# tatsuki1107/Relevance-FactorizationMachine

Hardware: AMD Instinct MI355X
Metric: training examples/sec (FM, k=32) (higher is better)
Workload: dtype f64; 1 GPU; kuairec_big: synthetic KuaiRec-big-shaped log 7176x10728 + 110 side-feature columns, n_features=18014, 15 nnz/row, N_train=1000000, FM k=32, IPS, lr=9e-06, batch_size=65536 rows per GPU (global 65536), step = gather+forward+residual+gradients+SGD update; row-id lists precomputed; batch_size_per_gpu=65536, global_batch=65536, parallelism=single

## Files before the change

relevance_factorizationmachine_amd/csrc/rfm_fm_kernels.hpp:

```cpp
#pragma once

#include <hip/amd_detail/amd_hip_unsafe_atomics.h>
#include <hip/hip_runtime.h>

#include <cstdint>
#include <type_traits>

#include "rfm_device_utils.hpp"
#include "rfm_fm_records.h"

namespace rfm {

template <int BLOCK>
__device__ inline double block_sum(double v, double* lds) {
  const int tid = threadIdx.x;
  __syncthreads();
  lds[tid] = v;
  __syncthreads();
#pragma unroll
  for (int s = BLOCK / 2; s > 0; s >>= 1) {
    if (tid < s) lds[tid] += lds[tid + s];
    __syncthreads();
  }
  return lds[0];
}

__device__ inline double logloss_term(double y, double p, double pred, double eps) {
  const double r = y / p;
  return r * log(pred + eps) + (1.0 - r) * log(1.0 - pred + eps);
}

constexpr int kBigBlock = 1024;
constexpr int kBigWaves = 4;
constexpr int kFwdRows = 2;

constexpr int kBigUnroll = 3;
constexpr int kSmallUnroll = 8;
constexpr int kSmallWideUnroll = 2;

constexpr int rows_in_flight(int nc) { return nc == 1 ? kFwdRows : 1; }
constexpr int kFwdRowsPlain = kFwdRows;
constexpr int kPlainUnroll = kBigUnroll;
constexpr int rows_in_flight_plain(int nc) { return nc == 1 ? kFwdRowsPlain : 1; }

constexpr bool hot_fixed_order(int lpr, int nc, int block, int rows) {
  return nc == 1 && (block / lpr) * rows <= 128;
}
constexpr int kHotUnroll = 2;
constexpr int kHotPosPad = 4;
inline size_t forward_lds_bytes(int block, int lpr, int vec, int nc, int rows, int n_hot, int k,
                                bool fixed_order) {
  size_t bytes = size_t(block) * 8 + (size_t(block) * rows + size_t(block / lpr)) * sizeof(Entry) +
                 size_t(n_hot) * size_t(k + 2) * 8;
  if (block == kBigBlock && n_hot == 0) bytes += 2 * size_t(block / lpr) * rows * 24;
  if (fixed_order && n_hot > 0 && hot_fixed_order(lpr, nc, block, rows)) {
    const size_t rt = size_t(block / lpr) * rows;
    bytes += rt * size_t(lpr * vec) * 8;
    if (rt / 32 > 1) bytes += size_t(block / lpr) * size_t(k + 2) * 8;
    bytes += ((size_t(n_hot) * ((rt + 31) / 32) + 1) & ~size_t(1)) * 4;
    bytes += (size_t(n_hot) * (rt + kHotPosPad) + 7) / 8 * 8;
  }
  return bytes;
}

struct FwdArgs {
  const Entry* ent;
  const RowRec* rows;
  const char* ell;
  int64_t ell_stride;
  const double2* ell_yp;
  const int64_t* indptr;
  const int32_t* indices;
  const double* values;
  const double* y;
  const double* pscore;
  const int32_t* row_ids;
  int64_t n_rows;
  int64_t n_rows_a;
  const int64_t* indptr2;
  const int32_t* indices2;
  const double* values2;
  const double* y2;
  const double* pscore2;
  double* loss_partial2;
  const double* w0;
  const double* w;
  const double* V;
  int32_t k;
  double* out_pred;
  double* out_err;
  double* out_Q;
  SlotMark* slot_mark;
  unsigned long long* slot_bits;
  int32_t n_hot;
  int32_t hot_rounds;
  int32_t hot_fixed;
  double* hot_slab;
  double* err_partial;
  double* loss_partial;
  double eps;
  int32_t grid_main;
  const int32_t* row_ids_x;
  int64_t n_rows_x;
  double* out_pred_x;
  int32_t grid_x;
  const RowRec* rows_y;
  const Entry* ent_y;
  int64_t n_rows_y;
  double* out_pred_y;
};

struct HotEnt {
  int32_t off;
  int32_t pad;
  double coef;
};
static_assert(sizeof(HotEnt) == sizeof(Entry), "HotEnt replaces an Entry in place");

template <int LPR, int VEC, int NC, int BLOCK, int R, bool REC, bool ELL = false, bool DET = false,
          bool SEG = false, bool XTRA = false>
__global__ __launch_bounds__(BLOCK, (BLOCK == kBigBlock ? kBigWaves : 1)) void fm_forward_kernel(
    FwdArgs a) {
  constexpr int GPB = BLOCK / LPR;
  unsigned bx = blockIdx.x, gx = gridDim.x;
  if constexpr (XTRA && REC) {
    if (int(blockIdx.x) >= a.grid_main) {
      const bool second = int(blockIdx.x) >= a.grid_main + a.grid_x;
      bx = blockIdx.x - a.grid_main - (second ? a.grid_x : 0);
      gx = second ? gridDim.x - a.grid_main - a.grid_x : a.grid_x;
      a.row_ids = second ? nullptr : a.row_ids_x;
      a.n_rows = second ? a.n_rows_y : a.n_rows_x;
      if (second) {
        a.rows = a.rows_y;
        a.ent = a.ent_y;
      }
      a.n_hot = 0;
      a.slot_mark = nullptr;
      a.slot_bits = nullptr;
      a.out_Q = nullptr;
      a.out_err = nullptr;
      a.err_partial = nullptr;
      a.loss_partial = nullptr;
      a.out_pred = second ? a.out_pred_y : a.out_pred_x;
    } else {
      gx = a.grid_main;
    }
  }
  constexpr bool seg = SEG && !REC;
  extern __shared__ double dyn_lds[];
  const int tid = threadIdx.x;
  const int l = tid % LPR;
  const int g = tid / LPR;
  const int k = a.k;
  const int hot_w = k + 2;
  const int H = a.n_hot;
  double* red = dyn_lds;
  Entry* ebuf = reinterpret_cast<Entry*>(dyn_lds + BLOCK) + g * (R * LPR + 1);
  double* hot = dyn_lds + BLOCK + 2 * (BLOCK * R + GPB);
  constexpr bool FIX = DET && REC && hot_fixed_order(LPR, NC, BLOCK, R);
  constexpr int RT = GPB * R;
  constexpr int KS = LPR * VEC;
  constexpr int NW = (RT + 31) / 32;
  constexpr int NCELL = RT / 32 > 1 ? RT / 32 : 1;
  constexpr int NHV = NCELL > 1 ? GPB / NCELL : 0;
  constexpr int PS = RT + kHotPosPad;
  double* Qs = hot + H * hot_w;
  double* part = Qs + RT * KS;
  unsigned int* hbits = reinterpret_cast<unsigned int*>(part + (NCELL > 1 ? GPB * hot_w : 0));
  uint8_t* hpos = reinterpret_cast<uint8_t*>(hbits + ((H * NW + 1) & ~1));
  const double w0 = a.w0[0];
  const int64_t last_row = a.n_rows - 1;
  double loss_acc = 0.0, loss_acc2 = 0.0, err_acc = 0.0;
  const bool stage_loss = BLOCK == kBigBlock && a.loss_partial != nullptr && H == 0;
  double* lstage = hot;
  int trip = 0;
  int fo[NC];
  bool fok[NC];
#pragma unroll
  for (int c = 0; c < NC; ++c) {
    const int f = (c * LPR + l) * VEC;
    fok[c] = f < k;
    fo[c] = fok[c] ? f : 0;
  }

  if (H > 0) {
    for (int i = tid; i < H * hot_w; i += BLOCK) hot[i] = 0.0;
    if (FIX)
      for (int i = tid; i < H * NW; i += BLOCK) hbits[i] = 0u;
    __syncthreads();
  }
  for (int64_t base = int64_t(bx) * (GPB * R); base < a.n_rows;
       base += int64_t(gx) * (GPB * R)) {
    int64_t t[R];
    int32_t r[R];
    using EntryOff = typename std::conditional<REC, int32_t, int64_t>::type;
    EntryOff p0[R];
    int len[R];
    double yy[R], pp[R];
    bool valid[R];
#pragma unroll
    for (int i = 0; i < R; ++i) {
      t[i] = base + i * GPB + g;
      valid[i] = t[i] <= last_row;
      r[i] = int32_t(valid[i] ? t[i] : last_row);
    }
    bool sb[R];
#pragma unroll
    for (int i = 0; i < R; ++i) sb[i] = seg && (valid[i] ? t[i] : last_row) >= a.n_rows_a;
    if (a.row_ids) {
#pragma unroll
      for (int i = 0; i < R; ++i) r[i] = a.row_ids[sb[i] ? 0 : r[i]];
    }
    if constexpr (seg) {
#pragma unroll
      for (int i = 0; i < R; ++i)
        if (sb[i]) r[i] = int32_t((valid[i] ? t[i] : last_row) - a.n_rows_a);
    }
    int32_t nxt[R];
    const int64_t nbase = base + int64_t(gx) * (GPB * R);
    constexpr bool ell = REC && ELL;
    const bool warm = ell && BLOCK == kBigBlock && a.row_ids && nbase < a.n_rows;
    int32_t* parked = reinterpret_cast<int32_t*>(red);
    if (warm) {
#pragma unroll
      for (int i = 0; i < R; ++i) {
        const int64_t nt = nbase + i * GPB + g;
        nxt[i] = a.row_ids[nt <= last_row ? nt : last_row];
      }
    }
    Entry e0[R];
    if (ell) {
#pragma unroll
      for (int i = 0; i < R; ++i) {
        e0[i] = reinterpret_cast<const Entry*>(a.ell + int64_t(r[i]) * a.ell_stride)[l];
        const double2 yp = a.ell_yp[r[i]];
        yy[i] = yp.x;
        pp[i] = yp.y;
        p0[i] = 0;
      }
      constexpr int GPW = kWave / LPR;
#pragma unroll
      for (int i = 0; i < R; ++i) {
        unsigned long long live = __ballot(e0[i].slot != kNilSlot);
        if (GPW > 1) live = (live >> ((g % GPW) * LPR)) & ((1ull << (LPR % 64)) - 1ull);
        len[i] = valid[i] ? __popcll(live) : 0;
      }
    }
#pragma unroll
    for (int i = 0; i < R; ++i) {
      if (ell) {
      } else if (REC) {
        const RowRec rec = a.rows[r[i]];
        p0[i] = EntryOff(rec.begin);
        len[i] = valid[i] ? int(rec.len) : 0;
        yy[i] = rec.y;
        pp[i] = rec.p;
      } else {
        const int64_t* ip = sb[i] ? a.indptr2 : a.indptr;
        const int64_t b0 = ip[r[i]], b1 = ip[r[i] + 1];
        p0[i] = EntryOff(b0);
        len[i] = valid[i] ? int(b1 - b0) : 0;
        yy[i] = 0.0;
        pp[i] = 1.0;
      }
    }
    if (!REC && a.y) {
#pragma unroll
      for (int i = 0; i < R; ++i) {
        yy[i] = (sb[i] ? a.y2 : a.y)[r[i]];
        pp[i] = (sb[i] ? a.pscore2 : a.pscore)[r[i]];
      }
    }
    int maxlen = len[0];
#pragma unroll
    for (int i = 1; i < R; ++i) maxlen = max(maxlen, len[i]);
    if (warm) {
#pragma unroll
      for (int i = 0; i < R; ++i)
        if (l == 0) parked[i * GPB + g] = nxt[i];
    }

    double q[R][NC][VEC];
    double s2[R], lin[R], err[R];
#pragma unroll
    for (int i = 0; i < R; ++i) {
      s2[i] = 0.0;
      lin[i] = 0.0;
      err[i] = 0.0;
#pragma unroll
      for (int c = 0; c < NC; ++c)
#pragma unroll
        for (int v = 0; v < VEC; ++v) q[i][c][v] = 0.0;
    }

    for (int pb = 0; pb < maxlen; pb += LPR) {
      Entry e[R];
#pragma unroll
      for (int i = 0; i < R; ++i) {
        const int my = pb + l;
        const EntryOff at = len[i] > 0 ? p0[i] + min(my, len[i] - 1) : 0;
        if (ell) {
          e[i] = e0[i];
        } else if (REC) {
          e[i] = a.ent[at];
        } else {
          e[i].col = (sb[i] ? a.indices2 : a.indices)[at];
          e[i].slot = 0;
          e[i].x = (sb[i] ? a.values2 : a.values)[at];
        }
        if (my >= len[i]) {
          e[i].slot = 0;
          e[i].x = 0.0;
        }
      }
#pragma unroll
      for (int i = 0; i < R; ++i) {
        lin[i] += a.w[e[i].col] * e[i].x;
        ebuf[i * LPR + l] = e[i];
      }
      const int cnt = (maxlen - pb) < LPR ? (maxlen - pb) : LPR;
#pragma unroll(BLOCK == kBigBlock || NC > 1 ? (NC == 1 && !DET && (ELL || !REC) ? (REC ? kBigUnroll : kPlainUnroll) : (BLOCK == kBigBlock || NC > 4 ? 2 : kSmallWideUnroll)) : kSmallUnroll)
      for (int j = 0; j < cnt; ++j) {
        Entry ej[R];
        Pack<VEC> pv[R][NC];
#pragma unroll
        for (int i = 0; i < R; ++i) {
          ej[i] = ebuf[i * LPR + j];
          const double* vrow = a.V + int64_t(ej[i].col) * k;
#pragma unroll
          for (int c = 0; c < NC; ++c) pv[i][c].load(vrow + fo[c]);
        }
#pragma unroll
        for (int i = 0; i < R; ++i) {
#pragma unroll
          for (int c = 0; c < NC; ++c) {
            const double xm = fok[c] ? ej[i].x : 0.0;
#pragma unroll
            for (int v = 0; v < VEC; ++v) {
              const double vx = pv[i][c].v[v] * xm;
              q[i][c][v] += vx;
              s2[i] += vx * vx;
            }
          }
        }
      }
    }

    if (warm) {
#pragma unroll
      for (int i = 0; i < R; ++i) nxt[i] = parked[i * GPB + g];
    }
#pragma unroll
    for (int i = 0; i < R; ++i) asm volatile("" ::"v"(yy[i]), "v"(pp[i]));
#pragma unroll
    for (int i = 0; i < R; ++i) {
      if (len[i] == 0) {
        s2[i] = 0.0;
        lin[i] = 0.0;
#pragma unroll
        for (int c = 0; c < NC; ++c)
#pragma unroll
          for (int v = 0; v < VEC; ++v) q[i][c][v] = 0.0;
      }
      double pair = -s2[i];
#pragma unroll
      for (int c = 0; c < NC; ++c)
#pragma unroll
        for (int v = 0; v < VEC; ++v) pair += q[i][c][v] * q[i][c][v];
      pair = group_sum<LPR>(pair);
      const double linsum = group_sum<LPR>(lin[i]);
      const double pred = sigmoid_clipped(w0 + linsum + 0.5 * pair);
      err[i] = valid[i] ? yy[i] / pp[i] - pred : 0.0;
      if (valid[i]) {
        if (a.out_Q) {
          const uint32_t qoff = uint32_t(t[i]) * uint32_t(k);
#pragma unroll
          for (int c = 0; c < NC; ++c) {
            if (fok[c]) {
              Pack<VEC> pq;
#pragma unroll
              for (int v = 0; v < VEC; ++v) pq.v[v] = q[i][c][v];
              if (REC)
                pq.store_through(a.out_Q + (qoff + uint32_t(fo[c])));
              else
                pq.store(a.out_Q + (qoff + uint32_t(fo[c])));
            }
          }
        }
        if (l == 0) {
          if (a.out_pred) a.out_pred[t[i]] = pred;
          if (a.out_err) a.out_err[t[i]] = err[i];
          if (a.loss_partial) {
            if (stage_loss) {
              double* st = lstage + ((trip & 1) * RT + i * GPB + g) * 3;
              st[0] = pred;
              st[1] = yy[i];
              st[2] = pp[i];
            } else if (sb[i]) {
              loss_acc2 += logloss_term(yy[i], pp[i], pred, a.eps);
            } else {
              loss_acc += logloss_term(yy[i], pp[i], pred, a.eps);
            }
          }
          err_acc += err[i];
        }
      } else if (stage_loss && l == 0) {
        lstage[((trip & 1) * RT + i * GPB + g) * 3] = -1.0;
      }
    }
    if (stage_loss) {
      __syncthreads();
      if (tid < RT) {
        const double* st = lstage + ((trip & 1) * RT + tid) * 3;
        if (!(st[0] < 0.0)) {
          const double term = logloss_term(st[1], st[2], st[0], a.eps);
          if (seg && base + tid >= a.n_rows_a)
            loss_acc2 += term;
          else
            loss_acc += term;
        }
      }
    }
    ++trip;

    int32_t touched[R];
    if (warm) {
#pragma unroll
      for (int i = 0; i < R; ++i)
        touched[i] = *reinterpret_cast<const int32_t*>(a.ell + int64_t(nxt[i]) * a.ell_stride +
                                                      16 * l);
    }
    if (REC && (a.slot_mark || H > 0)) {
      const bool fix_hot = FIX && H > 0;
      const int rounds_len = fix_hot ? a.hot_rounds * LPR : maxlen;
      for (int pb = 0; pb < rounds_len; pb += LPR) {
        Entry em[R];
#pragma unroll
        for (int i = 0; i < R; ++i) {
          if (rounds_len > LPR) {
            em[i] = a.ent[len[i] > 0 ? p0[i] + min(pb + l, len[i] - 1) : 0];
            if (pb + l >= len[i]) em[i] = Entry{0, 0, 0.0};
            if (FIX) ebuf[i * LPR + l] = em[i];
          } else {
            em[i] = ebuf[i * LPR + l];
          }
        }
        if (a.slot_mark) {
#pragma unroll
          for (int i = 0; i < R; ++i) {
            if (pb + l < len[i] && em[i].slot >= 0) {
              if (!DET) {
                Pack<2> pm;
                pm.v[0] = __hiloint2double(0, int32_t(t[i]));
                pm.v[1] = err[i];
                pm.store_through(reinterpret_cast<double*>(a.slot_mark + em[i].slot));
              } else {
                a.slot_mark[em[i].slot] = SlotMark{int32_t(t[i]), 0, err[i]};
              }
              atomicOr(a.slot_bits + (em[i].slot >> 6), 1ull << (em[i].slot & 63));
            }
          }
        }
        if (!(H > 0)) continue;
        if constexpr (FIX) {
#pragma unroll
          for (int i = 0; i < R; ++i) {
            const int row = i * GPB + g;
            if (pb == 0 && fok[0]) {
              Pack<VEC> pq;
#pragma unroll
              for (int v = 0; v < VEC; ++v) pq.v[v] = q[i][0][v];
              pq.store(Qs + row * KS + fo[0]);
            }
            const bool live = pb + l < len[i];
            if (live && em[i].slot < 0) {
              const int h = -1 - em[i].slot;
              atomicOr(&hbits[h * NW + (row >> 5)], 1u << (row & 31));
              hpos[h * PS + row] = uint8_t(l);
            }
            const double coef = live ? err[i] * em[i].x : 0.0;
            Pack<2> pc;
            pc.v[0] = coef;
            pc.v[1] = coef * em[i].x;
            pc.store(reinterpret_cast<double*>(ebuf + i * LPR + l));
          }
          __syncthreads();
          const Entry* ebase = reinterpret_cast<const Entry*>(dyn_lds + BLOCK);
          double acc[VEC], accw, accx;
          const auto add_rows = [&](int h, unsigned long long lo, unsigned long long hi, int base) {
            while (lo | hi) {
              constexpr int U = kHotUnroll;
              int rowu[U];
              bool ok[U];
#pragma unroll
              for (int u = 0; u < U; ++u) {
                ok[u] = (lo | hi) != 0;
                int bit = 0;
                if (lo) {
                  bit = __builtin_ctzll(lo);
                  lo &= lo - 1;
                } else if (hi) {
                  bit = 64 + __builtin_ctzll(hi);
                  hi &= hi - 1;
                }
                rowu[u] = base + bit;
              }
              int ju[U];
#pragma unroll
              for (int u = 0; u < U; ++u) ju[u] = hpos[h * PS + rowu[u]] & (LPR - 1);
              Pack<2> cf[U];
              Pack<VEC> qv[U];
#pragma unroll
              for (int u = 0; u < U; ++u) {
                const int gg = rowu[u] % GPB, ii = rowu[u] / GPB;
                cf[u].load(reinterpret_cast<const double*>(ebase + gg * (R * LPR + 1) + ii * LPR + ju[u]));
                qv[u].load(Qs + rowu[u] * KS + fo[0]);
              }
#pragma unroll
              for (int u = 0; u < U; ++u) {
                if (ok[u]) {
#pragma unroll
                  for (int v = 0; v < VEC; ++v) acc[v] += cf[u].v[0] * qv[u].v[v];
                  accw += cf[u].v[0];
                  accx += cf[u].v[1];
                }
              }
            }
          };
          const auto clear_acc = [&] {
#pragma unroll
            for (int v = 0; v < VEC; ++v) acc[v] = 0.0;
            accw = 0.0;
            accx = 0.0;
          };
          const auto add_to = [&](double* row_out, bool overwrite) {
            if (fok[0]) {
#pragma unroll
              for (int v = 0; v < VEC; ++v)
                row_out[fo[0] + v] = overwrite ? acc[v] : row_out[fo[0] + v] + acc[v];
            }
            if (l == 0) {
              row_out[k] = overwrite ? accw : row_out[k] + accw;
              row_out[k + 1] = overwrite ? accx : row_out[k + 1] + accx;
            }
          };
          if (NCELL > 1 && g / NCELL < H) {
            const int h = g / NCELL, cell = g % NCELL;
            const unsigned int word = hbits[h * NW + cell];
            if (l == 0) hbits[h * NW + cell] = 0u;
            clear_acc();
            add_rows(h, word, 0ull, cell * 32);
            add_to(part + g * hot_w, true);
          }
          for (int s2 = 0; NHV + s2 * GPB < H; ++s2) {
            const int h = NHV + s2 * GPB + ((s2 & 1) ? g : GPB - 1 - g);
            if (h >= H) continue;
            unsigned long long lo = 0, hi = 0;
#pragma unroll
            for (int wi = 0; wi < NW; ++wi) {
              const unsigned long long word = hbits[h * NW + wi];
              if (wi < 2)
                lo |= word << (32 * wi);
              else
                hi |= word << (32 * (wi - 2));
            }
            if ((lo | hi) == 0) continue;
            if (l < NW) hbits[h * NW + l] = 0u;
            clear_acc();
            add_rows(h, lo, hi, 0);
            add_to(hot + h * hot_w, false);
          }
          __syncthreads();
          if (NCELL > 1) {
            if (g < NHV && g < H) {
              double* hrow = hot + g * hot_w;
              for (int f = l; f < hot_w; f += LPR) {
                double sum = hrow[f];
#pragma unroll
                for (int c = 0; c < NCELL; ++c) sum += part[(g * NCELL + c) * hot_w + f];
                hrow[f] = sum;
              }
            }
          }
          continue;
        }
        const int cnt = (maxlen - pb) < LPR ? (maxlen - pb) : LPR;
        int wcnt = 0;
#pragma unroll
        for (int b = LPR; b > 0; b >>= 1)
          if (__ballot(cnt >= (wcnt | b))) wcnt |= b;
        const int rot = ((g % (kWave / LPR)) * wcnt) / (kWave / LPR);
        HotEnt* const hbuf = reinterpret_cast<HotEnt*>(ebuf);
        const int at = l - rot < 0 ? l - rot + wcnt : l - rot;
#pragma unroll
        for (int i = 0; i < R; ++i) {
          const bool on = pb + l < len[i] && em[i].slot < 0;
          const int off = on ? (-1 - em[i].slot) * hot_w : -1;
          const double coef = err[i] * em[i].x;
          if (l < wcnt) hbuf[i * LPR + at] = HotEnt{off, 0, coef};
          if (on) {
            double* const hsum = hot + (-em[i].slot * hot_w - 2);
            unsafeAtomicAdd(hsum, coef);
            unsafeAtomicAdd(hsum + 1, coef * em[i].x);
          }
        }
        for (int j = 0; j < wcnt; ++j) {
          HotEnt eh[R];
#pragma unroll
          for (int i = 0; i < R; ++i) eh[i] = hbuf[i * LPR + j];
          const bool pair01 = R == 2 && eh[0].off >= 0 && eh[0].off == eh[R - 1].off;
          const double coef2 = pair01 ? eh[R - 1].coef : 0.0;
          if (pair01) eh[R - 1].off = -1;
#pragma unroll
          for (int i = 0; i < R; ++i) {
#pragma unroll
            for (int c = 0; c < NC; ++c) {
              if (eh[i].off >= 0 && fok[c]) {
                double* hrow = hot + eh[i].off + fo[c];
#pragma unroll
                for (int v = 0; v < VEC; ++v)
                  unsafeAtomicAdd(hrow + v, R == 2 && i == 0
                                                ? eh[0].coef * q[0][c][v] + coef2 * q[R - 1][c][v]
                                                : eh[i].coef * q[i][c][v]);
              }
            }
          }
        }
      }
    }
    if (warm) {
#pragma unroll
      for (int i = 0; i < R; ++i) asm volatile("" ::"v"(touched[i]));
    }
  }

  if (H > 0) {
    __syncthreads();
    if constexpr (REC && VEC == 2) {
      for (int i = 2 * tid; i < H * hot_w; i += 2 * BLOCK) {
        const int h = i / hot_w, f = i % hot_w;
        Pack<2> ps;
        ps.load(hot + i);
        ps.store_through(a.hot_slab + (int64_t(h) * gx + bx) * hot_w + f);
      }
    } else {
      for (int i = tid; i < H * hot_w; i += BLOCK) {
        const int h = i / hot_w, f = i % hot_w;
        a.hot_slab[(int64_t(h) * gx + bx) * hot_w + f] = hot[i];
      }
    }
  }
  if (a.err_partial) {
    const double s = block_sum<BLOCK>(err_acc, red);
    if (tid == 0) a.err_partial[bx] = s;
  }
  if (a.loss_partial) {
    const double s = block_sum<BLOCK>(loss_acc, red);
    if (tid == 0) a.loss_partial[bx] = s;
  }
  if (seg && a.loss_partial2) {
    const double s = block_sum<BLOCK>(loss_acc2, red);
    if (tid == 0) a.loss_partial2[bx] = s;
  }
}

__global__ __launch_bounds__(kBlock) void loss_finish_kernel(const double* partial, int n_partial,
                                                            int64_t n_rows, double* out) {
  __shared__ double lds[kBlock];
  double acc = 0.0;
  for (int i = threadIdx.x; i < n_partial; i += kBlock) acc += partial[i];
  const double s = block_sum<kBlock>(acc, lds);
  if (threadIdx.x == 0) out[0] = -s / double(n_rows);
}

__global__ __launch_bounds__(kBlock) void loss_finish_many_kernel(const double* partial,
                                                                 int64_t stride, int n_partial,
                                                                 int64_t n_rows, double* out) {
  __shared__ double lds[kBlock];
  const double* row = partial + int64_t(blockIdx.x) * stride;
  double acc = 0.0;
  for (int i = threadIdx.x; i < n_partial; i += kBlock) acc += row[i];
  const double s = block_sum<kBlock>(acc, lds);
  if (threadIdx.x == 0) out[blockIdx.x] = -s / double(n_rows);
}

__global__ __launch_bounds__(kBlock) void logloss_kernel(const double* y, const double* pred,
                                                        const double* pscore,
                                                        const int32_t* row_ids, int64_t n_rows,
                                                        double eps, double* partial) {
  __shared__ double lds[kBlock];
  double acc = 0.0;
  for (int64_t t = int64_t(blockIdx.x) * kBlock + threadIdx.x; t < n_rows;
       t += int64_t(gridDim.x) * kBlock) {
    const int64_t r = row_ids ? int64_t(row_ids[t]) : t;
    acc += logloss_term(y[r], pscore[r], pred[t], eps);
  }
  const double s = block_sum<kBlock>(acc, lds);
  if (threadIdx.x == 0) partial[blockIdx.x] = s;
}

template <int U, class Rows>
__device__ inline void ordered_rows_sum(const Rows& from, int rows, int width,
                                        double* scratch , double* tot ) {
  const int fw = width < kBlock ? width : kBlock;
  const int nsg = kBlock / fw;
  const int sg = threadIdx.x / fw, fl = threadIdx.x % fw;
  const bool live = sg < nsg;
  for (int f0 = 0; f0 < width; f0 += fw) {
    const int f = f0 + fl;
    double acc = 0.0;
    if (live && f < width) {
      for (int r = sg; r < rows; r += nsg * U) {
        const double* row[U];
#pragma unroll
        for (int u = 0; u < U; ++u) row[u] = from.row(r + u * nsg < rows ? r + u * nsg : r);
        double v[U];
        bool ok[U];
#pragma unroll
        for (int u = 0; u < U; ++u) {
          v[u] = row[u][f];
          const bool counts = from.valid(row[u]);
          ok[u] = counts && r + u * nsg < rows;
        }
#pragma unroll
        for (int u = 0; u < U; ++u) acc += ok[u] ? v[u] : 0.0;
      }
    }
    __syncthreads();
    scratch[threadIdx.x] = acc;
    __syncthreads();
    if (sg == 0 && f < width) {
      double s = 0.0;
      for (int j = 0; j < nsg; ++j) s += scratch[j * fw + fl];
      tot[f] = s;
    }
  }
  __syncthreads();
}

struct SlabRows {
  const double* base;
  int width;
  __device__ const double* row(int r) const { return base + int64_t(r) * width; }
  __device__ bool valid(const double*) const { return true; }
};

struct PartRows {
  const double* parts;
  int first, k;
  double stamp;
  __device__ const double* row(int r) const { return parts + int64_t(first + r) * (k + 3); }
  __device__ bool valid(const double* row) const { return row[k + 2] == stamp; }
};

struct WinRec {
  int32_t t;
  int32_t col;
  double coef;
  double cx;
};

struct ColArgs {
  double* V;
  double* w;
  int32_t k;
  int64_t n;
  double lr;
  double* grad;
  int32_t* touch;
  int32_t touch_id;
  double* parts;
  double stamp;
};

struct ConsArgs {
  ColArgs c;
  const TaskRec* tasks;
  int32_t task_words;
  unsigned long long* slot_bits;
  unsigned long long* slot_bits_other;
  const SlotMark* slot_mark;
  const SlotRec* slots;
  const double* Q;
  double* w0;
  int32_t nb_tasks;
  int32_t n_hot;
  const int32_t* hot_cols;
  const double* hot_slab;
  int32_t n_slabs;
  const double* err_partial;
  int32_t n_chunks;
  int32_t xcd_chunks;
};

inline int fm_chunks(int k, int vec) { return ((k + vec - 1) / vec + 63) / 64; }

template <int VEC>
struct ColAcc {
  double m[VEC];
  double gw, d;
  __device__ inline void clear() {
#pragma unroll
    for (int v = 0; v < VEC; ++v) m[v] = 0.0;
    gw = 0.0;
    d = 0.0;
  }
  __device__ inline void store_row(double* row, int f, int k, bool scalars) const {
    if (f < k) {
#pragma unroll
      for (int v = 0; v < VEC; ++v) row[f + v] = m[v];
    }
    if (scalars) {
      row[k] = gw;
      row[k + 1] = d;
    }
  }
  __device__ inline void add_row(const double* row, int f, int k) {
    if (f < k) {
#pragma unroll
      for (int v = 0; v < VEC; ++v) m[v] += row[f + v];
    }
    gw += row[k];
    d += row[k + 1];
  }
  __device__ inline void load_row(const double* row, int fc, int k) {
#pragma unroll
    for (int v = 0; v < VEC; ++v) m[v] = row[fc + v];
    gw = row[k];
    d = row[k + 1];
  }
  __device__ inline void add_if(bool ok, const ColAcc& o) {
#pragma unroll
    for (int v = 0; v < VEC; ++v) m[v] += ok ? o.m[v] : 0.0;
    gw += ok ? o.gw : 0.0;
    d += ok ? o.d : 0.0;
  }
};

template <int VEC>
__device__ inline Pack<VEC> load_v_row(const double* V, int32_t col, int k, int f) {
  Pack<VEC> p;
  p.load(V + int64_t(col) * k + (f < k ? f : 0));
  return p;
}

__device__ inline double updated_factor(double vold, double m, double d, double lr, bool grad,
                                        bool dv_rounded) {
  double g;
  if (dv_rounded) {
#pragma clang fp contract(off)
    const double dv = d * vold;
    g = dv - m;
  } else {
    g = fma(d, vold, -m);
  }
  return grad ? g : fma(lr, -g, vold);
}

__device__ inline void add_by_only_writer(double* p, double x) { unsafeAtomicAdd(p, x); }

__device__ inline void apply_scalar(const ColArgs& c, double* p, int64_t at, double s) {
  if (c.grad)
    c.grad[c.n * c.k + at] = -s;
  else
    add_by_only_writer(p, c.lr * s);
}

__device__ inline void apply_w(const ColArgs& c, int32_t col, double gw) {
  apply_scalar(c, c.w + col, col, gw);
  if (c.grad && c.touch) c.touch[col] = c.touch_id;
}

template <int VEC>
__device__ inline void apply_column(const ColArgs& c, int32_t col, const ColAcc<VEC>& acc,
                                    const Pack<VEC>& vold, int f, bool scalars) {
  if (f < c.k) {
    Pack<VEC> out;
#pragma unroll
    for (int v = 0; v < VEC; ++v)
      out.v[v] = updated_factor(vold.v[v], acc.m[v], acc.d, c.lr, c.grad != nullptr, v == 0);
    out.store((c.grad ? c.grad : c.V) + int64_t(col) * c.k + f);
  }
  if (scalars) apply_w(c, col, acc.gw);
}

constexpr int kRowPre = (RFM_MAX_FACTORS + kBlock - 1) / kBlock;
__device__ inline void apply_column_block(const ColArgs& c, int32_t col, const double* tot,
                                          const double* vpre = nullptr) {
  const int k = c.k;
  const double gw = tot[k], d = tot[k + 1];
  int j = 0;
  for (int f = threadIdx.x; f < k; f += kBlock, ++j) {
    const int64_t at = int64_t(col) * k + f;
    const double vold = vpre ? vpre[j] : c.V[at];
    (c.grad ? c.grad : c.V)[at] = updated_factor(vold, tot[f], d, c.lr, c.grad != nullptr, false);
  }
  if (threadIdx.x == 0) apply_w(c, col, gw);
}

template <int LPR>
struct WinShape {
  static constexpr int PLANES = LPR >= 64 ? 1 : (LPR == 32 ? 2 : 4);
  static constexpr int WIN = PLANES * LPR;
  static constexpr int kGroupBytes = WIN * (int(sizeof(WinRec)) + 8);
};

constexpr int kConsHotBytes = (kBlock + 1024 + 2) * int(sizeof(double));
template <int LPR>
constexpr size_t consume_lds_bytes_of(int k) {
  constexpr size_t gpb = kBlock / LPR;
  const size_t tasks = gpb * WinShape<LPR>::kGroupBytes + gpb * size_t(k + 3) * sizeof(double);
  return tasks > size_t(kConsHotBytes) ? tasks : size_t(kConsHotBytes);
}
inline size_t consume_lds_bytes(int lpr, int k) {
  switch (lpr) {
    case 4: return consume_lds_bytes_of<4>(k);
    case 8: return consume_lds_bytes_of<8>(k);
    case 16: return consume_lds_bytes_of<16>(k);
    case 32: return consume_lds_bytes_of<32>(k);
    default: return consume_lds_bytes_of<64>(k);
  }
}

template <int LPR>
__device__ inline int group_scan(int v, int l) {
#pragma unroll
  for (int o = 1; o < LPR; o <<= 1) {
    const int up = __shfl_up(v, o, LPR);
    if (l >= o) v += up;
  }
  return v;
}

__device__ inline void consume_hot_column(const ConsArgs& a, int hb, double* lds) {
  const int k = a.c.k;
  const int32_t col = a.hot_cols[hb];
  double vpre[kRowPre];
#pragma unroll
  for (int j = 0; j < kRowPre; ++j) {
    const int f = int(threadIdx.x) + j * kBlock;
    vpre[j] = a.c.V[int64_t(col) * k + (f < k ? f : 0)];
  }
  double* tot = lds + kBlock;
  ordered_rows_sum<32>(SlabRows{a.hot_slab + int64_t(hb) * a.n_slabs * (k + 2), k + 2}, a.n_slabs,
                       k + 2, lds, tot);
  apply_column_block(a.c, col, tot, vpre);
}

__device__ inline void consume_w0(const ConsArgs& a, double* lds) {
  double acc = 0.0;
  for (int i = threadIdx.x; i < a.n_slabs; i += kBlock) acc += a.err_partial[i];
  const double s = block_sum<kBlock>(acc, lds);
  if (threadIdx.x == 0) apply_scalar(a.c, a.w0, a.c.n, s);
}

constexpr int kConsChBatch = 4;
template <int LPR, int VEC, bool CH = false>
__global__ __launch_bounds__(kBlock, 1) void fm_consume_kernel(ConsArgs a) {
  constexpr int GPB = kBlock / LPR;
  constexpr int PLANES = WinShape<LPR>::PLANES;
  constexpr int WIN = WinShape<LPR>::WIN;
  constexpr int BATCH = CH ? kConsChBatch : 4;
  int bx = int(blockIdx.x), chunk = 0;
  if (CH) {
    if (a.xcd_chunks) {
      const int xcd = bx & 7, slot = bx >> 3, nch = a.n_chunks;
      chunk = xcd * nch / 8;
      const int first = (chunk * 8 + nch - 1) / nch, next = ((chunk + 1) * 8 + nch - 1) / nch;
      bx = slot * (next - first) + (xcd - first);
      if (bx >= a.nb_tasks + a.n_hot + 1) return;
    } else {
      chunk = int(blockIdx.y);
    }
  }
  const int fb = chunk * (LPR * VEC);
  constexpr int TRIPS = kTaskTrips;
  constexpr int kGroupBytes = WinShape<LPR>::kGroupBytes;
  extern __shared__ double lds_raw[];
  const ColArgs& c = a.c;
  const int k = c.k;
  if (bx >= a.nb_tasks) {
    if (CH && chunk != 0) return;
    const int hb = bx - a.nb_tasks;
    if (hb < a.n_hot)
      consume_hot_column(a, hb, lds_raw);
    else
      consume_w0(a, lds_raw);
    return;
  }
  const int lane = threadIdx.x % kWave;
  const int l = lane % LPR;
  const int gb = threadIdx.x / LPR;
  const int f = fb + l * VEC;
  const bool scalars = l == 0 && fb == 0;
  const int task = bx * GPB + gb;
  const int W = a.task_words;
  const int32_t slot0 = task * W * 64;
  unsigned long long wd[TRIPS];
#pragma unroll
  for (int u = 0; u < TRIPS; ++u) {
    const int idx = u * LPR + l;
    wd[u] = idx < W ? a.slot_bits[int64_t(task) * W + idx] : 0ull;
  }
  const TaskRec tk = a.tasks[task];
#pragma unroll
  for (int u = 0; u < TRIPS; ++u) {
    if (CH) {
      if (fb == 0 && u * LPR + l < W) a.slot_bits_other[int64_t(task) * W + u * LPR + l] = 0ull;
    } else if (wd[u]) {
      a.slot_bits[int64_t(task) * W + u * LPR + l] = 0ull;
    }
  }

  char* gmem = reinterpret_cast<char*>(lds_raw) + gb * kGroupBytes;
  WinRec* wrec = reinterpret_cast<WinRec*>(gmem);
  int32_t* list = reinterpret_cast<int32_t*>(gmem + WIN * sizeof(WinRec));
  double* heads = reinterpret_cast<double*>(reinterpret_cast<char*>(lds_raw) + GPB * kGroupBytes);
  double* head = heads + gb * (k + 3);

  const bool head_open = tk.flags & 1;
  const bool tail_open = tk.flags & 2;
  ColAcc<VEC> acc;
  acc.clear();
  Pack<VEC> vold;
  int32_t cur = -1;
  int fill = 0;
  bool head_done = false;

  const auto finish = [&]() {
    if (head_open && cur == tk.first_col) {
      acc.store_row(head, f, k, l == 0);
      head_done = true;
    } else {
      apply_column(c, cur, acc, vold, f, scalars);
    }
  };

  const auto run_list = [&]() {
    SlotRec sr[PLANES];
    SlotMark mk[PLANES];
#pragma unroll
    for (int pl = 0; pl < PLANES; ++pl) {
      const int e = pl * LPR + l;
      const int32_t s = e < fill ? list[e] : slot0;
      mk[pl] = a.slot_mark[s];
      sr[pl] = a.slots[s];
    }
#pragma unroll
    for (int pl = 0; pl < PLANES; ++pl) {
      const int e = pl * LPR + l;
      if (e < fill) {
        const double coef = mk[pl].err * sr[pl].x;
        wrec[e] = WinRec{mk[pl].t, sr[pl].col, coef, coef * sr[pl].x};
      }
    }
    int at = 0;
    while (__ballot(at < fill)) {
      const int nb = max(min(BATCH, fill - at), 0);
      WinRec rec[BATCH];
      Pack<VEC> qq[BATCH], vv[BATCH];
#pragma unroll
      for (int u = 0; u < BATCH; ++u) {
        rec[u] = wrec[u < nb ? at + u : 0];
        if (u >= nb) {
          rec[u].t = 0;
          rec[u].col = 0;
        }
        qq[u].load(a.Q + int64_t(rec[u].t) * k + (f < k ? f : 0));
        if (rec[u].col != (u == 0 ? cur : rec[u > 0 ? u - 1 : 0].col))
          vv[u] = load_v_row<VEC>(c.V, rec[u].col, k, f);
      }
#pragma unroll
      for (int u = 0; u < BATCH; ++u) {
        if (u < nb) {
          if (rec[u].col != cur) {
            if (cur >= 0) finish();
            acc.clear();
            cur = rec[u].col;
            vold = vv[u];
          }
          const double coef = rec[u].coef, cx = rec[u].cx;
#pragma unroll
          for (int v = 0; v < VEC; ++v) acc.m[v] += coef * qq[u].v[v];
          acc.gw += coef;
          acc.d += cx;
        }
      }
      at += nb;
    }
    fill = 0;
  };

#pragma unroll
  for (int u = 0; u < TRIPS; ++u) {
    unsigned long long word = wd[u];
    const int32_t s0 = slot0 + (u * LPR + l) * 64;
    while (__ballot(word != 0ull)) {
      const int cnt = __popcll(word);
      const int before = group_scan<LPR>(cnt, l) - cnt;
      const int take = min(cnt, max(WIN - fill - before, 0));
      int pos = fill + before;
      for (int i = 0; i < take; ++i) {
        list[pos++] = s0 + (__ffsll((long long)word) - 1);
        word &= word - 1ull;
      }
      int added = take;
#pragma unroll
      for (int o = 1; o < LPR; o <<= 1) added += __shfl_xor(added, o, LPR);
      fill += added;
      if (__ballot(word != 0ull)) run_list();
    }
  }
  if (__ballot(fill > 0)) run_list();

  const bool through = head_open && tail_open && tk.first_col == tk.last_col;
  const bool own = (tail_open && !through) || tk.part >= 0;
  bool own_acc = false;
  if (cur >= 0) {
    if (own && cur == tk.last_col) {
      own_acc = true;
    } else {
      finish();
    }
  }
  if (head_open && l == 0) head[k + 2] = (head_done ? 1.0 : 0.0) + (through ? 2.0 : 0.0);
  if (!head_open && l == 0) head[k + 2] = 0.0;
  __syncthreads();
  if (own) {
    if (!own_acc) {
      acc.clear();
      vold = load_v_row<VEC>(c.V, tk.last_col, k, f);
    }
    bool any = own_acc;
    for (int g2 = gb + 1; g2 < GPB; ++g2) {
      const double* h2 = heads + g2 * (k + 3);
      const int fl = int(h2[k + 2]);
      if (fl & 1) {
        any = true;
        acc.add_row(h2, f, k);
      }
      if (!(fl & 2)) break;
    }
    if (tk.part >= 0) {
      double* row = c.parts + int64_t(tk.part) * (k + 3);
      acc.store_row(row, f, k, scalars);
      if (scalars) row[k + 2] = any ? c.stamp : 0.0;
    } else if (any) {
      apply_column(c, tk.last_col, acc, vold, f, scalars);
    }
  }
}

struct FinArgs {
  ColArgs c;
  const SplitCol* split;
  int32_t n_split_short;
  int32_t n_split_long;
};

template <int LPR, int VEC, int CB>
__device__ inline void finalize_short_columns(const FinArgs& a, int b, int fb) {
  constexpr int GPB = kBlock / LPR;
  const ColArgs& c = a.c;
  const int k = c.k;
  const int l = threadIdx.x % LPR;
  const int ci = b * GPB + threadIdx.x / LPR;
  if (ci >= a.n_split_short) return;
  const SplitCol cc = a.split[ci];
  const int f = fb + l * VEC;
  const int fc = f < k ? f : 0;
  ColAcc<VEC> acc;
  acc.clear();
  const Pack<VEC> vold = load_v_row<VEC>(c.V, cc.col, k, f);
  bool any = false;
  for (int i = 0; i < cc.part_count; i += CB) {
    ColAcc<VEC> part[CB];
    double ss[CB];
#pragma unroll
    for (int u = 0; u < CB; ++u) {
      const double* row = c.parts + int64_t(cc.part_begin + (i + u < cc.part_count ? i + u : i)) * (k + 3);
      part[u].load_row(row, fc, k);
      ss[u] = row[k + 2];
    }
#pragma unroll
    for (int u = 0; u < CB; ++u) {
      const bool ok = i + u < cc.part_count && ss[u] == c.stamp;
      any = any || ok;
      acc.add_if(ok, part[u]);
    }
  }
  if (any) apply_column(c, cc.col, acc, vold, f, l == 0 && fb == 0);
}

template <int LPR, int VEC>
__global__ __launch_bounds__(kBlock) void fm_finalize_kernel(FinArgs a, int nb_short) {
  __shared__ double scratch[kBlock];
  __shared__ double tot[1024 + 2];
  __shared__ int touched;
  const ColArgs& c = a.c;
  const int k = c.k;
  const int b = blockIdx.x;
  if (b < nb_short) return finalize_short_columns<LPR, VEC, 4>(a, b, 0);
  const SplitCol cc = a.split[a.n_split_short + (b - nb_short)];
  if (threadIdx.x == 0) touched = 0;
  __syncthreads();
  for (int r = threadIdx.x; r < cc.part_count; r += kBlock)
    if (c.parts[int64_t(cc.part_begin + r) * (k + 3) + k + 2] == c.stamp) touched = 1;
  __syncthreads();
  if (!touched) return;
  ordered_rows_sum<8>(PartRows{c.parts, cc.part_begin, k, c.stamp}, cc.part_count, k + 2, scratch, tot);
  apply_column_block(c, cc.col, tot);
}

template <int VEC>
__global__ __launch_bounds__(kBlock) void fm_finalize_chunk_kernel(FinArgs a, int nb_short) {
  constexpr int CW = kWave * VEC;
  __shared__ double tot[CW + 2];
  const ColArgs& c = a.c;
  const int k = c.k;
  const int b = blockIdx.x;
  const int fb = int(blockIdx.y) * CW;
  if (b < nb_short) {
    constexpr int LPR = kWave;
    constexpr int GPB = kBlock / LPR;
    constexpr int CB = 8;
    const int l = threadIdx.x % LPR;
    const int ci = b * GPB + threadIdx.x / LPR;
    if (ci >= a.n_split_short) return;
    const SplitCol cc = a.split[ci];
    const int f = fb + l * VEC;
    const int fc = f < k ? f : 0;
    ColAcc<VEC> acc;
    acc.clear();
    Pack<VEC> vold;
    vold.load(c.V + int64_t(cc.col) * k + fc);
    bool any = false;
    for (int i = 0; i < cc.part_count; i += CB) {
      Pack<VEC> mm[CB];
      double gg[CB], dd[CB], ss[CB];
#pragma unroll
      for (int u = 0; u < CB; ++u) {
        const double* row = c.parts + int64_t(cc.part_begin + (i + u < cc.part_count ? i + u : i)) * (k + 3);
        mm[u].load(row + fc);
        gg[u] = row[k];
        dd[u] = row[k + 1];
        ss[u] = row[k + 2];
      }
#pragma unroll
      for (int u = 0; u < CB; ++u) {
        const bool ok = i + u < cc.part_count && ss[u] == c.stamp;
        any = any || ok;
#pragma unroll
        for (int v = 0; v < VEC; ++v) acc.m[v] += ok ? mm[u].v[v] : 0.0;
        acc.gw += ok ? gg[u] : 0.0;
        acc.d += ok ? dd[u] : 0.0;
      }
    }
    if (any) apply_column(c, cc.col, acc, vold, f, l == 0 && fb == 0);
    return;
  }
  const SplitCol cc = a.split[a.n_split_short + (b - nb_short)];
  const int fcnt = k - fb < CW ? k - fb : CW;
  const int j = threadIdx.x;
  const bool live = j < fcnt + 2;
  const int cidx = j < fcnt ? fb + j : k + (j - fcnt);
  const double vold = c.V[int64_t(cc.col) * k + (j < fcnt ? fb + j : 0)];
  double acc = 0.0;
  bool any = false;
  constexpr int U = 32;
  for (int r0 = 0; r0 < cc.part_count; r0 += U) {
    double v[U], st[U];
#pragma unroll
    for (int u = 0; u < U; ++u) {
      const double* row = c.parts + int64_t(cc.part_begin + (r0 + u < cc.part_count ? r0 + u : r0)) * (k + 3);
      v[u] = row[live ? cidx : 0];
      st[u] = row[k + 2];
    }
#pragma unroll
    for (int u = 0; u < U; ++u) {
      const bool ok = r0 + u < cc.part_count && st[u] == c.stamp;
      any = any || ok;
      acc += ok ? v[u] : 0.0;
    }
  }
  if (!any) return;
  if (live) tot[j] = acc;
  __syncthreads();
  const double gw = tot[fcnt], d = tot[fcnt + 1];
  if (j < fcnt) {
    const int64_t at = int64_t(cc.col) * k + fb + j;
    if (c.grad)
      c.grad[at] = updated_factor(vold, acc, d, c.lr, true, false);
    else
      c.V[at] = updated_factor(vold, acc, d, c.lr, false, false);
  }
  if (j == 0 && fb == 0) {
    if (c.grad) {
      c.grad[c.n * k + cc.col] = -gw;
      if (c.touch) c.touch[cc.col] = c.touch_id;
    } else {
      add_by_only_writer(c.w + cc.col, c.lr * gw);
    }
  }
}

__global__ __launch_bounds__(kBlock) void ids_check_kernel(const int32_t* ids, int64_t batch,
                                                          int64_t n_iters, int64_t n_rows,
                                                          int32_t* seen, int32_t stamp0,
                                                          int32_t* flags) {
  const int64_t total = batch * n_iters;
  for (int64_t i = int64_t(blockIdx.x) * kBlock + threadIdx.x; i < total;
       i += int64_t(gridDim.x) * kBlock) {
    const int32_t r = ids[i];
    const int32_t stamp = stamp0 + int32_t(i / batch);
    if (r < 0 || r >= n_rows) {
      atomicOr(&flags[0], 1);
    } else if (atomicExch(&seen[r], stamp) == stamp) {
      atomicOr(&flags[1], 1);
    }
  }
}

__global__ __launch_bounds__(kBlock) void fm_apply_kernel(double* V, double* w, double* w0,
                                                         const double* grad, int64_t nk,
                                                         int64_t n, double lr) {
  const int64_t total = nk + n + 1;
  for (int64_t i = int64_t(blockIdx.x) * kBlock + threadIdx.x; i < total;
       i += int64_t(gridDim.x) * kBlock) {
    double* dst = i < nk ? V + i : (i < nk + n ? w + (i - nk) : w0);
    *dst -= lr * grad[i];
  }
}

}
```

Before: 1.312 billion examples/s.

## Accumulate hot-feature gradients with f64 MFMA tiles in non-deterministic path

Adds a tiled path for the non-deterministic hot-feature gradient accumulation (LPR=16, VEC=2, NC=1). Each group writes its coefficient for the first 16 hot ranks into an LDS strip, and the per-rank sums over rows are formed with f64 16x16x4 MFMA instructions. Only the reduced results are then added atomically into the hot table. Hot features with rank 16 or higher still go through the existing rotated per-entry atomic walk. The aim is to replace many contended LDS atomics with matrix-core reductions, at the cost of extra LDS, a wave-uniform loop condition and added code complexity.

New measurement: 1.400 billion examples/s (median of 6 runs). 1.07x the previous value.

```diff
diff --git a/relevance_factorizationmachine_amd/csrc/rfm_fm_kernels.hpp b/relevance_factorizationmachine_amd/csrc/rfm_fm_kernels.hpp
--- a/relevance_factorizationmachine_amd/csrc/rfm_fm_kernels.hpp
+++ b/relevance_factorizationmachine_amd/csrc/rfm_fm_kernels.hpp
@@ -46,6 +46,8 @@
 constexpr bool hot_fixed_order(int lpr, int nc, int block, int rows) {
   return nc == 1 && (block / lpr) * rows <= 128;
 }
+constexpr int kTileRanks = 16;
+constexpr bool hot_tile(int lpr, int vec, int nc) { return lpr == 16 && vec == 2 && nc == 1; }
 constexpr int kHotUnroll = 2;
 constexpr int kHotPosPad = 4;
 inline size_t forward_lds_bytes(int block, int lpr, int vec, int nc, int rows, int n_hot, int k,
@@ -53,6 +55,8 @@
   size_t bytes = size_t(block) * 8 + (size_t(block) * rows + size_t(block / lpr)) * sizeof(Entry) +
                  size_t(n_hot) * size_t(k + 2) * 8;
   if (block == kBigBlock && n_hot == 0) bytes += 2 * size_t(block / lpr) * rows * 24;
+  if (!fixed_order && n_hot > 0 && hot_tile(lpr, vec, nc))
+    bytes += size_t(block / lpr) * rows * kTileRanks * 8;
   if (fixed_order && n_hot > 0 && hot_fixed_order(lpr, nc, block, rows)) {
     const size_t rt = size_t(block / lpr) * rows;
     bytes += rt * size_t(lpr * vec) * 8;
@@ -165,6 +169,7 @@
   constexpr int NHV = NCELL > 1 ? GPB / NCELL : 0;
   constexpr int PS = RT + kHotPosPad;
   double* Qs = hot + H * hot_w;
+  constexpr bool TILE = REC && !DET && hot_tile(LPR, VEC, NC);
   double* part = Qs + RT * KS;
   unsigned int* hbits = reinterpret_cast<unsigned int*>(part + (NCELL > 1 ? GPB * hot_w : 0));
   uint8_t* hpos = reinterpret_cast<uint8_t*>(hbits + ((H * NW + 1) & ~1));
@@ -433,7 +438,7 @@
     if (REC && (a.slot_mark || H > 0)) {
       const bool fix_hot = FIX && H > 0;
       const int rounds_len = fix_hot ? a.hot_rounds * LPR : maxlen;
-      for (int pb = 0; pb < rounds_len; pb += LPR) {
+      for (int pb = 0; TILE ? __ballot(pb < rounds_len) != 0 : pb < rounds_len; pb += LPR) {
         Entry em[R];
 #pragma unroll
         for (int i = 0; i < R; ++i) {
@@ -579,6 +584,94 @@
 #pragma unroll
                 for (int c = 0; c < NCELL; ++c) sum += part[(g * NCELL + c) * hot_w + f];
                 hrow[f] = sum;
+              }
+            }
+          }
+          continue;
+        }
+        if constexpr (TILE) {
+          constexpr int GPW = kWave / LPR;
+          constexpr int NT = kTileRanks / 16;
+          typedef double tile_acc __attribute__((ext_vector_type(4)));
+          int tid_here = tid;
+          asm volatile("" : "+v"(tid_here));
+          const int lh = tid_here % LPR, gh = tid_here / LPR, gw = gh % GPW;
+          HotEnt* const hbuf = reinterpret_cast<HotEnt*>(ebuf);
+          double* const strip = hot + H * hot_w;
+          bool rowok[R], won[R];
+          unsigned long long walked[R];
+#pragma unroll
+          for (int i = 0; i < R; ++i) {
+            const bool live = pb + l < len[i] && em[i].slot < 0;
+            const int h = -1 - em[i].slot;
+            rowok[i] = valid[i] && __builtin_isfinite(err[i]);
+            const bool tile_e = live && rowok[i] && h < kTileRanks;
+            won[i] = live && !tile_e;
+            walked[i] = __ballot(won[i]);
+            const double coef = err[i] * em[i].x;
+            if (live) {
+              double* const hsum = hot + (-em[i].slot * hot_w - 2);
+              unsafeAtomicAdd(hsum, coef);
+              unsafeAtomicAdd(hsum + 1, coef * em[i].x);
+            }
+            double* const st = strip + (i * GPB + gh) * kTileRanks;
+#pragma unroll
+            for (int tl = 0; tl < NT; ++tl) st[tl * 16 + lh] = 0.0;
+            if (tile_e) st[h] = coef;
+          }
+          int wcnt = 0;
+#pragma unroll
+          for (int i = 0; i < R; ++i)
+#pragma unroll
+            for (int gq = 0; gq < GPW; ++gq)
+              wcnt = max(wcnt, __popc(unsigned(walked[i] >> (gq * LPR)) & ((1u << LPR) - 1u)));
+          const int rot = (gw * wcnt) / GPW;
+#pragma unroll
+          for (int i = 0; i < R; ++i) {
+            const unsigned bits = unsigned(walked[i] >> (gw * LPR)) & ((1u << LPR) - 1u);
+            const int below = __popc(bits & ((1u << lh) - 1u));
+            const int p = won[i] ? below : __popc(bits) + lh - below;
+            const int at = p - rot < 0 ? p - rot + wcnt : p - rot;
+            if (p < wcnt)
+              hbuf[i * LPR + at] = HotEnt{won[i] ? (-1 - em[i].slot) * hot_w : -1, 0, err[i] * em[i].x};
+          }
+#pragma unroll
+          for (int v = 0; v < VEC; ++v) {
+            tile_acc D[NT];
+#pragma unroll
+            for (int tl = 0; tl < NT; ++tl) D[tl] = tile_acc{0.0, 0.0, 0.0, 0.0};
+#pragma unroll
+            for (int i = 0; i < R; ++i) {
+              const double* const st = strip + (i * GPB + gh) * kTileRanks;
+              const double b = rowok[i] ? q[i][0][v] : 0.0;
+#pragma unroll
+              for (int tl = 0; tl < NT; ++tl)
+                D[tl] = __builtin_amdgcn_mfma_f64_16x16x4f64(st[tl * 16 + lh], b, D[tl], 0, 0, 0);
+            }
+#pragma unroll
+            for (int tl = 0; tl < NT; ++tl)
+#pragma unroll
+              for (int reg = 0; reg < 4; ++reg) {
+                const int rank = tl * 16 + gw + 4 * reg;
+                if (rank < H && fok[0]) unsafeAtomicAdd(hot + rank * hot_w + fo[0] + v, D[tl][reg]);
+              }
+          }
+          for (int j = 0; j < wcnt; ++j) {
+            HotEnt eh[R];
+#pragma unroll
+            for (int i = 0; i < R; ++i) eh[i] = hbuf[i * LPR + j];
+            const bool pair01 = R == 2 && eh[0].off >= 0 && eh[0].off == eh[R - 1].off;
+            const double coef2 = pair01 ? eh[R - 1].coef : 0.0;
+            if (pair01) eh[R - 1].off = -1;
+#pragma unroll
+            for (int i = 0; i < R; ++i) {
+              if (eh[i].off >= 0 && fok[0]) {
+                double* hrow = hot + eh[i].off + fo[0];
+#pragma unroll
+                for (int v = 0; v < VEC; ++v)
+                  unsafeAtomicAdd(hrow + v, R == 2 && i == 0
+                                                ? eh[0].coef * q[0][0][v] + coef2 * q[R - 1][0][v]
+                                                : eh[i].coef * q[i][0][v]);
               }
             }
           }
```
